# zabaras/deep-turbulence

Measured on AMD Instinct MI355X. Metric: flow-field samples/sec (fwd+log-det+bwd), 64x256x256x4; optimizer step: HipAdam (one-launch Adam, same update as torch.optim.Adam), higher is better.
Workload: dtype f32

## Files before the change

deep-turbulence_amd/csrc/tmg_common.h:

```cpp
#pragma once
#include <hip/hip_runtime.h>
#include <stdint.h>
#include <stdlib.h>
#include <atomic>

typedef float f32x4 __attribute__((ext_vector_type(4)));

__device__ __forceinline__ __amdgpu_buffer_rsrc_t tmg_make_rsrc(const void* base, unsigned bytes) {
    return __builtin_amdgcn_make_buffer_rsrc(const_cast<void*>(base), 0, (int)bytes, 0x00020000);
}
__device__ __forceinline__ float4 tmg_bload4(__amdgpu_buffer_rsrc_t rs, unsigned voff, unsigned soff) {
    const f32x4 v = __builtin_bit_cast(f32x4, __builtin_amdgcn_raw_buffer_load_b128(rs, (int)voff, (int)soff, 0));
    return make_float4(v[0], v[1], v[2], v[3]);
}

#define TMG_MAX_IN_SEG 3
#define TMG_MAX_OUT_SEG 3

struct TmgSeg {
    const float* p;
    int stride;
    int off;
    int n;
};
// ... 289 lines not shown
static inline int tmg_persistent_grid(int gy, int ntiles) {
    const int g = tmg_num_cus() / gy;
    return g > ntiles ? ntiles : (g < 1 ? 1 : g);
}

struct TmgSegList { int csum; bool vec4; };
template <typename SEG, typename PTRS>
static inline TmgSegList tmg_decode_segs(SEG* dst, int slots, PTRS ptrs, const int64_t* desc, int64_t n) {
    TmgSegList r{0, true};
    for (int i = 0; i < slots; ++i) {
        if (i >= n) { dst[i] = SEG{nullptr, 0, 0, 0}; continue; }
        dst[i] = SEG{(decltype(dst[i].p))ptrs[i], (int)desc[3 * i], (int)desc[3 * i + 1], (int)desc[3 * i + 2]};
        if (((dst[i].stride | dst[i].off | dst[i].n) & 3) || (((uintptr_t)ptrs[i]) & 15)) r.vec4 = false;
        r.csum += dst[i].n;
    }
    return r;
}
static inline TmgSegList tmg_decode_in(TmgSeg* dst, const void* const* ptrs, const int64_t* desc, int64_t n, int slots = TMG_MAX_IN_SEG) {
    return tmg_decode_segs(dst, slots, ptrs, desc, n);
}
static inline TmgSegList tmg_decode_out(TmgOSeg* dst, void* const* ptrs, const int64_t* desc, int64_t n, int slots = TMG_MAX_OUT_SEG) {
    return tmg_decode_segs(dst, slots, ptrs, desc, n);
}
static inline bool tmg_bad_seg_count(int64_t nin, int64_t nout) {
    return nin < 1 || nin > TMG_MAX_IN_SEG || nout < 1 || nout > TMG_MAX_OUT_SEG;
}
struct TmgD2 { int stride, off; };
static inline TmgD2 tmg_opt_d2(const void* p, const int64_t* d) { return p ? TmgD2{(int)d[0], (int)d[1]} : TmgD2{0, 0}; }

#define TMG_CHECK_LAUNCH()                          \
    do {                                            \
        hipError_t e__ = hipGetLastError();         \
        if (e__ != hipSuccess) return (int)e__;     \
    } while (0)
```

deep-turbulence_amd/csrc/tmg_conv.hip:

```cpp
#include "tmg_common.h"
#include <stdlib.h>

static __device__ float g_tmg_zero_page[64];

struct ConvP {
    TmgSeg in[TMG_MAX_IN_SEG];
    int nseg;
    int vec4;
    int B, Hin, Win, Hout, Wout;
    int ksize, stride;
    int Cin, Cin_pad, Cout, Cout_pad;
    const float* wpk;
    const float* bias;
    const float* kappa;
    const float* in_scale;
    const float* in_shift;
    int relu_in, pad_rep, relu_out, accumulate;
    TmgOSeg out[TMG_MAX_OUT_SEG];
    int nout;
    TmgSeg add;
    int TW_log2, TH;
    int KCH;
    int tiles_x, tiles_y;
    int ntiles, nchunks;
    int ovec4;
};

template <int MT, int NTW, int WM, int WN>
__global__ __launch_bounds__(256) void conv_mfma_kernel(ConvP p) {
    extern __shared__ __attribute__((aligned(16))) float lds[];
    const int tid = threadIdx.x, lane = tid & 63, wave = tid >> 6;
    const int wm = wave % WM, wn = wave / WM;
    const int li = lane & 15, q = lane >> 4;
    constexpr int MBLK = 16 * MT * WM;

    int t = blockIdx.x;
    const int tx = t % p.tiles_x;
    t /= p.tiles_x;
    const int ty = t % p.tiles_y;
    const int b = t / p.tiles_y;
    const int TWl = p.TW_log2, TW = 1 << TWl, TH = MBLK >> TWl;
    const int oy0 = ty * TH, ox0 = tx * TW;
    const int s = p.stride, halo = p.ksize >> 1;
    const int PW = s * (TW - 1) + 1 + 2 * halo, PH = s * (TH - 1) + 1 + 2 * halo;
    const int iy0 = s * oy0 - halo, ix0 = s * ox0 - halo;
    const int ntaps = p.ksize * p.ksize;
    const int KB = p.Cin_pad >> 4;

// ... 334 lines not shown
                if (store_only) {
#pragma unroll
                    for (int i = 0; i < MT; ++i) {
                        const int oy = oy0_ + (mrc[i] >> 16), ox = ox0_ + (mrc[i] & 0xffff);
                        if (oy < p.Hout && ox < p.Wout) {
                            const unsigned opx = (unsigned)(__umul24(b_ * p.Hout + oy, p.Wout) + ox);
#pragma unroll
                            for (int j = 0; j < NTW; ++j) {
                                const int n0 = (ntile0 + j) * 16 + 4 * qe;
                                if (n0 < p.Cout) {
                                    float v[4] = {acc[i][j][0], acc[i][j][1], acc[i][j][2], acc[i][j][3]};
                                    if (HB) { v[0] += biasq[HB ? j : 0].x; v[1] += biasq[HB ? j : 0].y; v[2] += biasq[HB ? j : 0].z; v[3] += biasq[HB ? j : 0].w; }
                                    if (PREADD && p.add.p) {
                                        const float4 a4 = addv[PREADD ? i : 0][PREADD ? j : 0];
                                        v[0] += a4.x; v[1] += a4.y; v[2] += a4.z; v[3] += a4.w;
                                    }
#pragma unroll
                                    for (int r = 0; r < 4; ++r) {
                                        v[r] *= osc;
                                        if (p.relu_out) v[r] = fmaxf(v[r], 0.f);
                                    }
                                    int nl = n0;
                                    TMG_PICK_OSEG(p.out, nl, op_, ostride, ooff)
                                    *reinterpret_cast<float4*>(op_ + (size_t)opx * (unsigned)ostride + ooff + nl) = make_float4(v[0], v[1], v[2], v[3]);
                                }
                            }
                        }
                    }
                } else
#pragma unroll
                for (int i = 0; i < MT; ++i) {
                    const int oy = oy0_ + (mrc[i] >> 16), ox = ox0_ + (mrc[i] & 0xffff);
                    if (oy < p.Hout && ox < p.Wout) {
                        const unsigned opx = (unsigned)(__umul24(b_ * p.Hout + oy, p.Wout) + ox);
#pragma unroll
                        for (int j = 0; j < NTW; ++j) {
                            const int n0 = (ntile0 + j) * 16 + 4 * qe;
                            if (n0 < p.Cout) {
                                float v[4] = {acc[i][j][0], acc[i][j][1], acc[i][j][2], acc[i][j][3]};
                                if (HB) {
                                    v[0] += biasq[HB ? j : 0].x; v[1] += biasq[HB ? j : 0].y; v[2] += biasq[HB ? j : 0].z; v[3] += biasq[HB ? j : 0].w;
                                } else if (p.bias) {
#pragma unroll
                                    for (int r = 0; r < 4; ++r) v[r] += (n0 + r < p.Cout) ? p.bias[n0 + r] : 0.f;
                                }
                                if (p.ovec4) {
                                    int nl = n0;
                                    TMG_PICK_OSEG(p.out, nl, op_, ostride, ooff)
                                    float4* dst = reinterpret_cast<float4*>(op_ + (size_t)opx * (unsigned)ostride + ooff + nl);
                                    if (p.add.p) {
                                        const float4 a4 = (PREADD) ? addv[PREADD ? i : 0][PREADD ? j : 0]
                                                                   : *reinterpret_cast<const float4*>(p.add.p + (size_t)opx * (unsigned)p.add.stride + p.add.off + n0);
                                        v[0] += a4.x; v[1] += a4.y; v[2] += a4.z; v[3] += a4.w;
                                    }
#pragma unroll
                                    for (int r = 0; r < 4; ++r) {
                                        v[r] *= osc;
                                        if (p.relu_out) v[r] = fmaxf(v[r], 0.f);
                                    }
                                    if (p.accumulate) {
                                        const float4 o4 = *dst;
                                        v[0] += o4.x; v[1] += o4.y; v[2] += o4.z; v[3] += o4.w;
                                    }
                                    *dst = make_float4(v[0], v[1], v[2], v[3]);
                                } else {
#pragma unroll
                                    for (int r = 0; r < 4; ++r) {
                                        const int n = n0 + r;
                                        if (n < p.Cout) {
                                            int nl = n;
                                            TMG_PICK_OSEG(p.out, nl, op_, ostride, ooff)
// ... 903 lines not shown
}

template <int MT, int NTW, int WM, int WN>
static int launch_fwd(const ConvP& p, int G, int gy, size_t lds_bytes, hipStream_t st, int64_t* plan) {
    if (plan) { fill_fwd_plan(plan, 0, MT, NTW, WM, WN, p, G, gy, lds_bytes); return 0; }
    TMG_LDS_OPTIN((&conv_fwd_kernel<MT, NTW, WM, WN>));
    const int kid = p.ksize == 1 ? 31 : 11 + (WM == 8 ? NTW - 1 : (WM == 4 ? NTW + 1 : NTW + 3));
    ProfScope prof(kid, 2.0 * p.B * p.Hout * p.Wout * (double)p.Cout * p.Cin * p.ksize * p.ksize, st);
    hipLaunchKernelGGL((conv_fwd_kernel<MT, NTW, WM, WN>), dim3(G, gy, 1), dim3(512), lds_bytes, st, p);
    TMG_CHECK_LAUNCH();
    return 0;
}

static int conv_fwd_lean(ConvP p, hipStream_t st, int64_t* plan) {
    if (p.stride != 1 || !p.vec4 || (p.Cin & 3) || (long)p.Hin * p.Win >= (1 << 24) || (long)p.B * p.Hout >= (1 << 24) ||
        p.Wout >= (1 << 24) || (long)p.B * p.Hout * p.Wout >= (1L << 32))
        return -100;
    for (int i = 0; i < p.nseg; ++i)
        if (p.in[i].stride >= (1 << 24) || (long)p.B * p.Hin * p.Win * p.in[i].stride >= (1L << 31)) return -100;
    p.ovec4 = (p.Cout & 3) == 0;
    for (int i = 0; i < p.nout; ++i)
        if (((p.out[i].stride | p.out[i].off | p.out[i].n) & 3) || (((uintptr_t)p.out[i].p) & 15)) p.ovec4 = 0;
    if (p.add.p && (((p.add.stride | p.add.off) & 3) || (((uintptr_t)p.add.p) & 15))) p.ovec4 = 0;
    const int ntt = p.Cout_pad >> 4;
    int WM, WN, NTW;
    if (ntt <= 4) { WM = 8; WN = 1; NTW = ntt; }
    else if (ntt <= 8) { WM = 4; WN = 2; NTW = ntt <= 6 ? 3 : 4; }
    else { WM = 2; WN = 4; NTW = ntt <= 12 ? 3 : 4; }
    const int gy = (ntt + WN * NTW - 1) / (WN * NTW);
    const long npix = (long)p.B * p.Hout * p.Wout;
    const int halo = p.ksize >> 1;
    for (int MT = 4; MT >= 1; MT >>= 1) {
        if (MT > 1 && (npix / (16 * MT * WM)) * gy < 256) continue;
        const int MBLK = 16 * MT * WM;
        int twl = ilog2_ceil(p.Wout);
        if (twl > 5) twl = 5;
        if (twl < 2) twl = 2;
        while ((1 << twl) > MBLK) --twl;
        while (twl < 5 && (MBLK >> twl) > p.Hout && (1 << twl) < p.Wout) ++twl;
        const int TW = 1 << twl, TH = MBLK >> twl;
        if (TH < 1) continue;
        const int PHPW = (TW + 2 * halo) * (TH + 2 * halo);
        int nchunks = (p.Cin_pad + 63) / 64, kch = 0;
        for (; nchunks <= p.Cin_pad / 16; ++nchunks) {
            kch = (((p.Cin_pad / 16) + nchunks - 1) / nchunks) * 16;
            const int k4p = kch <= 16 ? 4 : (kch <= 32 ? 8 : 16);
// ... 95 lines not shown

static int conv_fwd_impl(const void* const* in_ptrs, const int64_t* in_desc, int64_t nseg, const void* wpk, const void* bias,
                         const void* kappa, const void* in_scale, const void* in_shift, const void* add,
                         const int64_t* add_desc, void* const* out_ptrs, const int64_t* out_desc, int64_t nout,
                         const int64_t* dims, hipStream_t st, int64_t* plan) {
    ConvP p;
    const TmgD2 ad = tmg_opt_d2(add, add_desc);
    p.add = TmgSeg{(const float*)add, ad.stride, ad.off, 0};
    p.nseg = (int)nseg;
    const TmgSegList si = tmg_decode_in(p.in, in_ptrs, in_desc, nseg);
    p.vec4 = si.vec4;
    p.B = (int)dims[0]; p.Hin = (int)dims[1]; p.Win = (int)dims[2]; p.Hout = (int)dims[3]; p.Wout = (int)dims[4];
    p.ksize = (int)dims[5]; p.stride = (int)dims[6]; p.Cin = (int)dims[7]; p.Cout = (int)dims[8];
    p.relu_in = (int)dims[9]; p.pad_rep = (int)dims[10]; p.relu_out = (int)dims[11]; p.accumulate = (int)dims[12];
    if (p.ksize != 1 && p.ksize != 3) return -2;
    if (si.csum != p.Cin || tmg_bad_seg_count(nseg, nout)) return -3;
    p.Cin_pad = (p.Cin + 15) & ~15;
    p.Cout_pad = (p.Cout + 15) & ~15;
    p.wpk = (const float*)wpk; p.bias = (const float*)bias; p.kappa = (const float*)kappa;
    p.in_scale = (const float*)in_scale; p.in_shift = (const float*)in_shift;
    p.nout = (int)nout;
    if (tmg_decode_out(p.out, out_ptrs, out_desc, nout).csum != p.Cout) return -4;

    {
        const int rc = conv_fwd_lean(p, st, plan);
        if (rc != -100) return rc;
    }

    const int ntt = p.Cout_pad >> 4;
    int WM, WN, NTW;
    if (ntt <= 4) { WM = 4; WN = 1; NTW = ntt; }
    else if (ntt <= 6) { WM = 2; WN = 2; NTW = 3; }
    else if (ntt <= 8) { WM = 2; WN = 2; NTW = 4; }
    else if (ntt <= 12) { WM = 1; WN = 4; NTW = 3; }
    else { WM = 1; WN = 4; NTW = 4; }
    const int gy = (ntt + WN * NTW - 1) / (WN * NTW);
    int MT = 4;
    while (MT > 1) {
        const long npix = (long)p.B * p.Hout * p.Wout;
        if ((npix / (16 * MT * WM)) * gy >= 512) break;
        MT >>= 1;
    }
    const int MBLK = 16 * MT * WM;
    int twl = ilog2_ceil(p.Wout);
    if (twl > 5) twl = 5;
    if (twl < 2) twl = 2;
    while ((1 << twl) > MBLK) --twl;
    while (twl < 5 && (MBLK >> twl) > p.Hout && (1 << twl) < p.Wout) ++twl;
    p.TW_log2 = twl;
    const int TW = 1 << twl;
// ... 365 lines not shown
```

deep-turbulence_amd/csrc/tmg_wino.hip:

```cpp
#include "tmg_common.h"
#include <stdlib.h>
#include <type_traits>

struct WinoP {
    TmgSeg in[TMG_MAX_IN_SEG];
    int nseg;
    int B, Hin, Win;
    int Cin, Cin_pad, Cout, Npad;
    const float* U;
    const float* bias;
    int relu_in, pad_rep;
    TmgOSeg out[TMG_MAX_OUT_SEG];
    int tiles_x, tiles_y, ntiles;
    int nchunks;
};

__global__ void wino_pack_kernel(const float* __restrict__ w, float* __restrict__ U, int Cout, int Cin, int K, int N, int Kpad, int Npad, int mode) {
    const size_t total = (size_t)Kpad * Npad;
    for (size_t i = blockIdx.x * (size_t)blockDim.x + threadIdx.x; i < total; i += (size_t)gridDim.x * blockDim.x) {
        const int c16 = i & 15;
        size_t r = i >> 4;
        const int n = r % Npad;
        const int kb = r / Npad;
        const int k = kb * 16 + c16;
        float g[3][3];
#pragma unroll
        for (int a = 0; a < 3; ++a)
#pragma unroll
            for (int b = 0; b < 3; ++b) {
                float v = 0.f;
                if (k < K && n < N) v = mode == 0 ? w[((size_t)n * Cin + k) * 9 + a * 3 + b] : w[((size_t)k * Cin + n) * 9 + (2 - a) * 3 + (2 - b)];
                g[a][b] = v;
            }
        float t[4][3];
#pragma unroll
// ... 242 lines not shown
                    TMG_WN_POSITION
                };
#define TMG_WN_P(I) one_position(std::integral_constant<int, I>{});
                TMG_WN_P(0) TMG_WN_P(1) TMG_WN_P(2) TMG_WN_P(3) TMG_WN_P(4) TMG_WN_P(5) TMG_WN_P(6) TMG_WN_P(7)
                TMG_WN_P(8) TMG_WN_P(9) TMG_WN_P(10) TMG_WN_P(11) TMG_WN_P(12) TMG_WN_P(13) TMG_WN_P(14) TMG_WN_P(15)
#undef TMG_WN_P
#undef TMG_WN_LOADB
            }
            if (cm + 1 == nchunks) {
                int t_ = tm;
                const int tx_ = t_ % p.tiles_x; t_ /= p.tiles_x;
                const int ty_ = t_ % p.tiles_y;
                const int b_ = t_ / p.tiles_y;
#pragma unroll
                for (int m = 0; m < 2; ++m) {
                    const int wt = 16 * m + li;
                    const int oyb = ty_ * TH + 2 * (wt >> 3), oxb = tx_ * TW + 2 * (wt & 7);
#pragma unroll
                    for (int n = 0; n < NPW; ++n) {
                        const int n0 = (ntile0 + n) * 16 + 4 * q;
                        if (ntile0 + n < ntt && n0 < p.Cout) {
                            int nl = n0;
                            TMG_PICK_OSEG(p.out, nl, optr, ostride, ooff)
#pragma unroll
                            for (int o = 0; o < 4; ++o) {
                                const int oy = oyb + (o >> 1), ox = oxb + (o & 1);
                                if (oy < p.Hin && ox < p.Win) {
                                    const unsigned opx = ((unsigned)b_ * (unsigned)p.Hin + (unsigned)oy) * (unsigned)p.Win + (unsigned)ox;
                                    *reinterpret_cast<float4*>(optr + (size_t)opx * (unsigned)ostride + ooff + nl) =
                                        make_float4(Y[o][m][n][0], Y[o][m][n][1], Y[o][m][n][2], Y[o][m][n][3]);
                                }
                            }
                        }
                    }
                }
#pragma unroll
                for (int o = 0; o < 4; ++o)
#pragma unroll
                    for (int m = 0; m < 2; ++m)
#pragma unroll
                        for (int n = 0; n < NPW; ++n) Y[o][m][n] = bvr[n];
                cm = 0; tm += G;
            } else {
                ++cm;
            }
        }
// ... 151 lines not shown
                    af[0][m] = v4[(pos * VPL + m * 16 * VS) / 4];
                    af[1][m] = v4[(pos * VPL + m * 16 * VS + 16) / 4];
                }
                __builtin_amdgcn_sched_barrier(0);
                TMG_WN_POSITION
            }
        }
#undef TMG_WN_LOADB
        if (cm + 1 == nchunks) {
            int t_ = tm;
            const int tx_ = t_ % p.tiles_x; t_ /= p.tiles_x;
            const int ty_ = t_ % p.tiles_y;
            const int b_ = t_ / p.tiles_y;
#pragma unroll
            for (int m = 0; m < 2; ++m) {
                const int wt = 16 * m + li;
                const int oyb = ty_ * TH + 2 * (wt >> 3), oxb = tx_ * TW + 2 * (wt & 7);
#pragma unroll
                for (int n = 0; n < NPW; ++n) {
                    const int n0 = (ntile0 + n) * 16 + 4 * q;
                    if (ntile0 + n < ntt && n0 < p.Cout) {
                        int nl = n0;
                        TMG_PICK_OSEG(p.out, nl, optr, ostride, ooff)
#pragma unroll
                        for (int o = 0; o < 4; ++o) {
                            const int oy = oyb + (o >> 1), ox = oxb + (o & 1);
                            if (oy < p.Hin && ox < p.Win) {
                                const unsigned opx = ((unsigned)b_ * (unsigned)p.Hin + (unsigned)oy) * (unsigned)p.Win + (unsigned)ox;
                                *reinterpret_cast<float4*>(optr + (size_t)opx * (unsigned)ostride + ooff + nl) =
                                    make_float4(Y[o][m][n][0], Y[o][m][n][1], Y[o][m][n][2], Y[o][m][n][3]);
                            }
                        }
                    }
                }
            }
#pragma unroll
            for (int o = 0; o < 4; ++o)
#pragma unroll
                for (int m = 0; m < 2; ++m)
#pragma unroll
                    for (int n = 0; n < NPW; ++n) Y[o][m][n] = bvr[n];
            cm = 0; tm += G;
        } else {
            ++cm;
        }
    }
}

template <typename P>
static int wino_fwd_setup(P& p, const void* const* in_ptrs, const int64_t* in_desc, int64_t nseg, const void* U, const void* bias,
                          void* const* out_ptrs, const int64_t* out_desc, int64_t nout, const int64_t* dims, int cin_granule, bool narrow) {
    p.nseg = (int)nseg;
    if (tmg_bad_seg_count(nseg, nout)) return -3;
    const TmgSegList si = tmg_decode_in(p.in, in_ptrs, in_desc, nseg), so = tmg_decode_out(p.out, out_ptrs, out_desc, nout);
    p.B = (int)dims[0]; p.Hin = (int)dims[1]; p.Win = (int)dims[2]; p.Cin = (int)dims[3]; p.Cout = (int)dims[4];
    p.relu_in = (int)dims[5]; p.pad_rep = (int)dims[6];
    if (si.csum != p.Cin || so.csum != p.Cout) return -3;
    bool ok = si.vec4 && so.vec4 && !(p.Cout & 3) && !(p.Cin & 3);
    if (narrow ? (p.Cout > 48 || p.Cin < 64) : p.Cout < 64) ok = false;
    if (bias && (((uintptr_t)bias) & 15)) ok = false;
    if (!ok) return -100;
    p.Cin_pad = (p.Cin + cin_granule - 1) & ~(cin_granule - 1);
    p.Npad = (p.Cout + 15) & ~15;
    p.U = (const float*)U; p.bias = (const float*)bias;
    p.tiles_x = (p.Win + 15) / 16; p.tiles_y = (p.Hin + 7) / 8;
    p.ntiles = p.B * p.tiles_x * p.tiles_y;
    p.nchunks = (p.Cin_pad + 31) / 32;
    if (p.ntiles <= 0) return 0;
    if ((long long)p.B * p.Hin * p.Win >= (1LL << 31)) return -100;
    return 1;
}

#define TMG_WINO_FWD_PLAN_N 13
template <typename P>
static void fill_wino_fwd_plan(int64_t* plan, int kernel, int npw, const P& p, int gx, int gy, size_t lds_bytes) {
    const int64_t v[TMG_WINO_FWD_PLAN_N] = {kernel, npw, p.Cin_pad, p.nchunks, (p.Cin_pad - 32 * (p.nchunks - 1) + 15) / 16, p.Npad / 16, p.tiles_x,
                                            p.tiles_y, p.ntiles, gx, gy, (p.ntiles + gx - 1) / gx, (int64_t)lds_bytes};
    for (int i = 0; i < TMG_WINO_FWD_PLAN_N; ++i) plan[i] = v[i];
}

// ... 317 lines not shown
                for (int m = 0; m < 2; ++m)
#pragma unroll
                    for (int n = 0; n < NPW; ++n) TMG_W3_YUPD(15, m, n)
#undef TMG_W3_YUPD
#undef TMG_W3_LOADB
            }
            if (cm + 1 == nch) {
                int t_ = tm;
                const int tx_ = t_ % p.tiles_x; t_ /= p.tiles_x;
                const int ty_ = t_ % p.tiles_y;
                const int b_ = t_ / p.tiles_y;
                int lie = li, qe = q;
                asm volatile("" : "+v"(lie), "+v"(qe));
#pragma unroll
                for (int m = 0; m < 2; ++m) {
                    const int wt = 16 * m + lie;
                    const int oyb = ty_ * TH + 2 * (wt >> 3), oxb = tx_ * TW + 2 * (wt & 7);
#pragma unroll
                    for (int n = 0; n < NPW; ++n) {
                        const int n0 = (ntile0 + n) * 16 + 4 * qe;
                        if (ntile0 + n < ntt && n0 < p.Cout) {
                            int nl = n0;
                            TMG_PICK_OSEG(p.out, nl, optr, ostride, ooff)
#pragma unroll
                            for (int o = 0; o < 4; ++o) {
                                const int oy = oyb + (o >> 1), ox = oxb + (o & 1);
                                if (oy < p.Hin && ox < p.Win) {
                                    const unsigned opx = ((unsigned)b_ * (unsigned)p.Hin + (unsigned)oy) * (unsigned)p.Win + (unsigned)ox;
                                    __builtin_nontemporal_store(Y[o][m][n],
                                                                reinterpret_cast<f32x4*>(optr + (size_t)opx * (unsigned)ostride + ooff + nl));
                                }
                            }
                        }
                    }
                }
#pragma unroll
                for (int o = 0; o < 4; ++o)
#pragma unroll
                    for (int m = 0; m < 2; ++m)
#pragma unroll
                        for (int n = 0; n < NPW; ++n) Y[o][m][n] = bvr[n];
                cm = 0; tm += G;
            } else {
                ++cm;
            }
        }
// ... 767 lines not shown
```

deep-turbulence_amd/tmg_hip.py:

```python
import ctypes
import os
import weakref
import subprocess
import sys

import torch

_HERE = os.path.dirname(os.path.abspath(__file__))
LIB_PATH = os.path.join(_HERE, "libtmglow_hip.so")
CSRC = os.path.join(_HERE, "csrc")
SOURCES = ["tmg_conv.hip", "tmg_pointwise.hip", "tmg_physics.hip", "tmg_mix16.hip", "tmg_coupling.hip", "tmg_wino.hip", "tmg_thin.hip", "tmg_glue.hip", "tmg_ensemble.hip", "tmg_spectrum.hip", "tmg_scores.hip", "tmg_tspec.hip", "tmg_quant.hip", "tmg_gram.hip", "tmg_sfun.hip", "tmg_event.hip", "tmg_pdf.hip", "tmg_pod.hip", "tmg_phase.hip", "tmg_spod.hip"]
NO_PACKED_F32 = ["tmg_wino.hip", "tmg_conv.hip", "tmg_coupling.hip", "tmg_thin.hip", "tmg_mix16.hip", "tmg_spectrum.hip", "tmg_tspec.hip",
                 "tmg_pod.hip", "tmg_spod.hip"]
_lib = None

c_i64 = ctypes.c_int64
c_vp = ctypes.c_void_p

EXPORTS = [
    "tmg_conv_pack", "tmg_conv_pack_map", "tmg_conv_fwd", "tmg_conv_fwd_add", "tmg_affine_bwd_scaled", "tmg_c1_fwd_add", "tmg_conv_wgrad", "tmg_conv_wgrad_ws_floats", "tmg_conv_rep_border_fix", "tmg_conv_dgrad_direct",
    "tmg_affine_apply", "tmg_affine_apply_pass", "tmg_bn_finalize", "tmg_affine_bwd", "tmg_lstm_pointwise_fwd", "tmg_lstm_pointwise_bwd", "tmg_gauss_fwd",
    "tmg_gauss_bwd", "tmg_checker", "tmg_upsample_fwd", "tmg_upsample_bwd", "tmg_chan_reduce", "tmg_bn_bwd_apply",
    "tmg_phys_fwd", "tmg_phys_rms", "tmg_phys_bwd", "tmg_conv_wgrad_grouped", "tmg_conv_wgrad_grouped_ws_floats", "tmg_conv_pack_batched", "tmg_masked_add", "tmg_c1x2_fwd", "tmg_c1_fwd", "tmg_c1_bwd", "tmg_dense2_bwd", "tmg_dkappa", "tmg_prof_enable", "tmg_prof_collect", "tmg_mix_f16", "tmg_phys_bwd_dev", "tmg_coupling_fwd", "tmg_coupling_bwd",
    "tmg_conv_wino_pack", "tmg_conv_wino_fwd", "tmg_conv_wino_narrow", "tmg_conv_wino_wgrad", "tmg_conv_wino_wgrad_ws_floats", "tmg_mix_f32", "tmg_lu_fold_fwd", "tmg_lu_fold_bwd", "tmg_lu_fold_bwd_split", "tmg_level_finish", "tmg_conv_wgrad_thin_grouped", "tmg_mix_wgrad_grouped", "tmg_layer_planes", "tmg_conv_wino_wgrad_grouped", "tmg_conv_wino_wgrad_grouped_ws_floats", "tmg_adam_step", "tmg_chan_moments", "tmg_bn_finalize64", "tmg_mix_f32_affine_fwd", "tmg_mix_f32_affine_bwd", "tmg_conv_pack_many", "tmg_pad_halves", "tmg_coupling_fwd_halves", "tmg_coupling_bwd_halves", "tmg_fill_i64", "tmg_conv_wino_pack3", "tmg_conv_wino_fwd3", "tmg_mat_inverse", "tmg_gauss_sample", "tmg_reverse_loss_fwd", "tmg_reverse_loss_bwd", "tmg_sum_terms", "tmg_vec_sum", "tmg_level_pack", "tmg_spread2", "tmg_phys_fields", "tmg_phys_fields_bwd",
# ... 141 lines not shown
    if t.is_cuda and t.device.index != torch.cuda.current_device():
        raise RuntimeError("TM-Glow HIP op called with a tensor on %s while the current device is cuda:%d: wrap the call in "
                           "`with torch.cuda.device(t.device):` (or torch.cuda.set_device once per process)"
                           % (t.device, torch.cuda.current_device()))


def nhwc(x):
    check_act(x)
    check_device(x)
    return x.permute(0, 2, 3, 1).contiguous()


def nchw(t):
    return t.permute(0, 3, 1, 2)


def _segs(tensors):
    d = [seg(t) for t in tensors]
    ptrs = (c_vp * len(d))(*[x[0] for x in d])
    desc = (c_i64 * (3 * len(d)))(*[v for x in d for v in (x[1], x[2], x[3])])
    return ptrs, desc, len(d)


def _d2(t):
    return (c_i64 * 2)(seg(t)[1] if t is not None else 0, 0)


def _i64(*v):
    return (c_i64 * len(v))(*[int(x) for x in v])


def _flts(vals):
    return (ctypes.c_float * len(vals))(*[float(v) for v in vals])


def _launched(rc, name):
    if rc == -100:
        return False
    _chk(rc, name)
    return True


def _packed_numel(mode, ce, Cout, k):
    K, N = (ce, Cout) if mode == 0 else (Cout, ce)
    return k * k * ((K + 15) // 16 * 16) * ((N + 15) // 16 * 16)

# ... 79 lines not shown
        op = (c_vp * len(ws))(*[v.data_ptr() for v in views])
        _chk(lib().tmg_conv_pack_many(wp, op, _i64(*desc), c_i64(len(ws)), _stream()), "tmg_conv_pack_many")
        outs += views
    return outs


def conv_pack_batched(w, mode, cin_eff=0, cmap=None):
    check_act(w)
    w = w.contiguous()
    N_, Cout, Cin, k, _ = w.shape
    ce = int(cin_eff) if cmap is not None else max(int(cin_eff), Cin)
    wpk = torch.empty((N_, _packed_numel(mode, ce, Cout, k)), device=w.device, dtype=torch.float32)
    m = cmap if cmap is not None else (Cin, 0x7fffffff, 0)
    _chk(lib().tmg_conv_pack_batched(_ptr(w), _ptr(wpk), c_i64(N_), c_i64(Cout), c_i64(Cin), c_i64(ce), c_i64(k), c_i64(mode), _i64(*m),
                                     _stream()), "tmg_conv_pack_batched")
    return wpk


def conv_fwd(inputs, wpk, Cout, ksize, stride, outs, bias=None, kappa=None, in_scale=None, in_shift=None, relu_in=False,
             pad_rep=False, relu_out=False, accumulate=False, add=None):
    B, Hin, Win, _ = inputs[0].shape
    Hout, Wout = outs[0].shape[1], outs[0].shape[2]
    ip, idesc, n_in = _segs(inputs)
    op, odesc, n_out = _segs(outs)
    Cin = sum(t.shape[3] for t in inputs)
    assert sum(t.shape[3] for t in outs) == Cout
    dims = _i64(B, Hin, Win, Hout, Wout, ksize, stride, Cin, Cout, relu_in, pad_rep, relu_out, accumulate)
    if add is not None:
        _chk(lib().tmg_conv_fwd_add(ip, idesc, c_i64(n_in), _ptr(wpk), _ptr(bias), _ptr(kappa), _ptr(in_scale), _ptr(in_shift), _ptr(add),
                                    _d2(add), op, odesc, c_i64(n_out), dims, _stream()), "tmg_conv_fwd_add")
        return
    _chk(lib().tmg_conv_fwd(ip, idesc, c_i64(n_in), _ptr(wpk), _ptr(bias), _ptr(kappa), _ptr(in_scale), _ptr(in_shift), op, odesc,
                            c_i64(n_out), dims, _stream()), "tmg_conv_fwd")


def wino_eligible(Cin, Cout, ksize, stride):
    return ksize == 3 and stride == 1 and Cout >= 64 and Cout % 4 == 0 and Cin % 4 == 0 and Cin >= 16


def wino_narrow_eligible(Cin, Cout):
    return Cout <= 48 and Cout % 4 == 0 and Cin % 4 == 0 and Cin >= 64


def conv_wino_pack(w, mode=0, nvalid=0):
    Cout, Cin = w.shape[0], w.shape[1]
    assert w.shape[2] == 3 and w.shape[3] == 3
    w = w.contiguous()
# ... 7 lines not shown


def set_winograd_precision(kind):
    if kind not in ("f32", "bf16x3"):
        raise ValueError("Winograd precision must be 'f32' or 'bf16x3', got %r" % (kind,))
    _WINO_PRECISION[0] = kind


def winograd_precision():
    return _WINO_PRECISION[0]


def conv_wino_pack3(w, mode=0, nvalid=0):
    Cout, Cin = w.shape[0], w.shape[1]
    assert w.shape[2] == 3 and w.shape[3] == 3
    w = w.contiguous()
    K, N = (Cin, Cout) if mode == 0 else (Cout, nvalid if 0 < nvalid < Cin else Cin)
    U = torch.empty(16 * ((K + 31) // 32 * 32) * ((N + 15) // 16 * 16) * 3, device=w.device, dtype=torch.int16)
    _chk(lib().tmg_conv_wino_pack3(_ptr(w), _ptr(U), c_i64(Cout), c_i64(Cin), c_i64(mode), c_i64(nvalid), _stream()), "tmg_conv_wino_pack3")
    return U


def _wino_fwd(name, inputs, U, Cout, outs, bias, *flags):
    if isinstance(outs, torch.Tensor):
        outs = [outs]
    B, Hin, Win, _ = inputs[0].shape
    ip, idesc, n_in = _segs(inputs)
    op, odesc, n_out = _segs(outs)
    Cin = sum(t.shape[3] for t in inputs)
    assert sum(t.shape[3] for t in outs) == Cout and outs[0].shape[1] == Hin and outs[0].shape[2] == Win
    return _launched(getattr(lib(), name)(ip, idesc, c_i64(n_in), _ptr(U), _ptr(bias), op, odesc, c_i64(n_out),
                                          _i64(B, Hin, Win, Cin, Cout, *flags), _stream()), name)


def conv_wino_fwd3(inputs, U, Cout, outs, bias=None, relu_in=False, pad_rep=False):
    return _wino_fwd("tmg_conv_wino_fwd3", inputs, U, Cout, outs, bias, relu_in, pad_rep)


def conv_wino_narrow(inputs, U, Cout, outs, bias=None, relu_in=False, pad_rep=False, relu_out=False):
    return _wino_fwd("tmg_conv_wino_narrow", inputs, U, Cout, outs, bias, relu_in, pad_rep, relu_out)


def conv_wino_fwd(inputs, U, Cout, outs, bias=None, relu_in=False, pad_rep=False):
    return _wino_fwd("tmg_conv_wino_fwd", inputs, U, Cout, outs, bias, relu_in, pad_rep)


def conv3x3_auto(inputs, weight, Cout, outs, bias=None, relu_in=False, pad_rep=False, relu_out=False, dgrad=False, nvalid=0):
    Cin = sum(t.shape[3] for t in inputs)
    mode = 1 if dgrad else 0
    if not relu_out and wino_eligible(Cin, Cout, 3, 1):
        if (_WINO_PRECISION[0] == "bf16x3"
                and conv_wino_fwd3(inputs, conv_wino_pack3(weight, mode, nvalid), Cout, outs, bias=bias, relu_in=relu_in, pad_rep=pad_rep)):
            return None
        if conv_wino_fwd(inputs, conv_wino_pack(weight, mode, nvalid), Cout, outs, bias=bias, relu_in=relu_in, pad_rep=pad_rep):
            return None
    if wino_narrow_eligible(Cin, Cout):
        if conv_wino_narrow(inputs, conv_wino_pack(weight, mode, nvalid), Cout, outs, bias=bias, relu_in=relu_in, pad_rep=pad_rep,
                            relu_out=relu_out):
            return None
    wpk = conv_pack(weight, mode, nvalid, (nvalid, 1 << 30, 0)) if (dgrad and nvalid) else conv_pack(weight, mode)
    conv_fwd(inputs, wpk, Cout, 3, 1, outs, bias=bias, relu_in=relu_in, pad_rep=pad_rep, relu_out=relu_out)
    return wpk


_WS = {}


def workspace(nfloats, device):
    if torch.cuda.is_current_stream_capturing():
        return torch.empty(max(int(nfloats), 1), device=device, dtype=torch.float32)
    key = (device.index, torch._C._cuda_getCurrentRawStream(torch._C._cuda_getDevice()))
    buf = _WS.get(key)
    if buf is None or buf.numel() < nfloats:
        buf = torch.empty(max(int(nfloats), 1 << 20), device=device, dtype=torch.float32)
        _WS[key] = buf
    return buf


_WINO_WGRAD_CIN_MIN = 32
# ... 1011 lines not shown
```

deep-turbulence_amd/tmg_ops.py:

```python
import collections
import math
import numbers

import os
import threading
import weakref

import torch

import tmg_hip as H

LOG5 = math.log(5.0)
LOG4 = math.log(4.0)
SPLIT_LIMITS = (-2.0, LOG5, -2.0, LOG5)
TOP_LIMITS = (0.0, 0.0, -10.0, LOG5)


class _ZeroPool:
    CHUNK = 8 << 20
    LIMIT = 2 << 20

    def __init__(self):
        self.lock = threading.Lock()
        self.cur = {}
# ... 908 lines not shown
    return dx


_Level = collections.namedtuple("_Level", "NL NLp C ch Cc cin reverse fuse split rec w1s w2s wzs bzs kps")
_LevelBwd = collections.namedtuple("_LevelBwd", "g Wm PZt PMt DH DD quad_last grouped zc_kw wg_in mix_wg dWz dBz dW1 dW2 dWm dbm DDp")


def _level(wts, C, Cc, reverse):
    NL = len(wts) // 5
    ch = C // 2
    fuse = 8 <= C <= 32 and ch % 4 == 0 and all(w.is_contiguous() for w in wts)
    split = fuse and reverse and C in (16, 32)
    rec = _RECOMPUTE[0] and fuse and reverse and C <= 64
    return _Level(NL, (NL + 3) // 4 * 4, C, ch, Cc, ch + Cc, reverse, fuse, split, rec,
                  wts[0::5], wts[1::5], wts[2::5], wts[3::5], wts[4::5])


class LevelCouplingFn(torch.autograd.Function):

    @staticmethod
    def _cond_parts(L, cond, Wcat):
        bhw, dev = cond.shape[:3], cond.device
        Wzc, Wdc = Wcat[:L.NL * L.C], Wcat[L.NL * L.C:]
        Hc = empty(bhw + (L.NL * L.C,), dev)
        H.conv3x3_auto([cond], Wzc, L.NL * L.C, [Hc], relu_in=True, pad_rep=True)
        Dc = empty(bhw + (2 * L.NLp,), dev)
        H.conv_fwd([cond], H.conv_pack(Wdc, 0), 2 * L.NLp, 3, 1, [Dc], relu_in=True)
        if math.prod(bhw) >= int(os.environ.get("TMG_LAYER_PLANES_MIN", 1 << 17)):
            Dc = H.layer_planes(Dc)
            dc_of = lambda k: (Dc[k][..., 0:1], Dc[k][..., 1:2])
        else:
            dc_of = lambda k: (Dc[..., 2 * k:2 * k + 1], Dc[..., 2 * k + 1:2 * k + 2])
        return Hc, Dc, dc_of

    @staticmethod
    def _level_operands(L, dev):
        NL, NLp, C, ch, Cc, cin = L[:6]
        layers = list(zip(L.w1s, L.w2s, L.wzs, L.bzs, L.kps))
        Wz = empty((NL, C, cin + 2, 3, 3), dev)
        Wcat = empty((NL * C + 2 * NLp, Cc, 3, 3), dev)
        Bz = empty((NL, C), dev)
        Kp = empty(NL, dev)
        if all(w.is_contiguous() and w.dtype == torch.float32 for ws in layers for w in ws) and os.environ.get("TMG_NO_LEVEL_PACK") is None:
            tab = H._segment_table([[w.data_ptr() for w in ws] for ws in layers], dev)
            H.level_pack(tab, Wz, Wcat, Bz, Kp, NL, NLp, C, ch, Cc)
            return Wz, Wcat, Bz, Kp
        torch.stack(L.wzs, out=Wz)
        Wcat[:NL * C] = Wz[:, :, ch:cin].reshape(NL * C, Cc, 3, 3)
        Wdc = Wcat[NL * C:].view(NLp, 2, Cc, 3, 3)
        Wdc[NL:].zero_()
        Wdc[:NL, 0] = torch.stack(L.w1s)[:, 0, ch:cin]
        Wdc[:NL, 1] = torch.stack(L.w2s)[:, 0, ch:cin]
        torch.stack(L.bzs, out=Bz)
        torch.stack([kp.reshape(()) for kp in L.kps], out=Kp)
        return Wz, Wcat, Bz, Kp

    @staticmethod
    def _growth(L, k, x1, dc_of):
        D = empty(x1.shape[:3] + (4,), x1.device)
        add1, add2 = dc_of(k)
        H.c1x2_fwd([x1], L.w1s[k], L.w2s[k], D, w_rows=L.ch, w2_d1_row=L.cin, add1=add1, add2=add2)
        return D

    @staticmethod
    def _fwd_fused(L, k, cur, Wm, bm, PM, Hc, dc_of, logdet):
        C, ch, reverse = L.C, L.ch, L.reverse
        bhw, dev = Hc.shape[:3], Hc.device
        tin = cur if reverse else _mix_fwd(cur, Wm[k], bm[k], PM[k])
        t1 = H._halves(tin)[0]
        D = LevelCouplingFn._growth(L, k, t1, dc_of)
        if L.split and k != 0:
            out = (empty(bhw + (ch,), dev), empty(bhw + (ch,), dev))
        else:
            out = empty(bhw + (C,), dev)
        r = empty(bhw + (ch,), dev)
        y2 = empty(bhw + (ch,), dev) if reverse else None
        ok = H.coupling_fwd(tin, out, r, y2, D, Hc[..., k * C:(k + 1) * C], L.wzs[k], L.bzs[k], L.kps[k], Wm[k] if reverse else None,
                            bm[k] if reverse else None, logdet, reverse, L.cin)
        assert ok
        if L.rec:
            return out, None
        return out, ((tin, D, r, [t1, y2]) if reverse else (tin, D, r, out, cur))

    @staticmethod
    def _fwd_wide(L, k, cur, Wm, bm, PM, PZ, Hc, dc_of, logdet, mixaff):
        C, ch, reverse = L.C, L.ch, L.reverse
        bhw, dev = Hc.shape[:3], Hc.device
        tin = cur if reverse else _mix_fwd(cur, Wm[k], bm[k], PM[k])
        x1 = tin[..., :ch]
        if ch % 4 == 0:
            D = LevelCouplingFn._growth(L, k, x1, dc_of)
        else:
            D = empty(bhw + (4,), dev)
            add1, add2 = dc_of(k)
            H.c1_fwd([x1], L.w1s[k], D[..., 0:1], relu_in=True, w_rows=ch, fill4=True, add=add1)
            H.c1_fwd([x1, D], L.w2s[k], D[..., 1:2], relu_in=True, w_rows=ch + 1, w_split=ch, w_gap=L.Cc, add=add2)
        hh = empty(bhw + (C,), dev)
        H.conv_fwd([x1, D], PZ[k], C, 3, 1, [hh], bias=L.bzs[k], kappa=L.kps[k], relu_in=True, pad_rep=True, add=Hc[..., k * C:(k + 1) * C])
        r = empty(bhw + (ch,), dev)
        if mixaff:
            y2 = empty(bhw + (ch,), dev)
            out = empty(bhw + (C,), dev)
            if H.mix_affine_fwd(tin, hh, Wm[k], bm[k], out, r, y2, logdet):
                return out, (tin, D, r, [x1, y2])
        y = empty(bhw + (C,), dev)
        H.affine_apply(hh, tin[..., ch:], y[..., ch:], r, logdet, reverse, x1=x1, y1=y[..., :ch])
        return (_mix_fwd(y, Wm[k], bm[k], PM[k]) if reverse else y), (tin, D, r, y) + (() if reverse else (cur,))

    @staticmethod
    def forward(ctx, x, cond, Wm, bm, reverse, *wts):
        x = x if x.stride(3) == 1 else x.contiguous()
        cond = cond.contiguous()
        L = _level(wts, x.shape[3], cond.shape[3], reverse)
        NL, C, ch = L.NL, L.C, L.ch
        dev = x.device
        Wz, Wcat, Bz, Kp = LevelCouplingFn._level_operands(L, dev)
        Hc, Dc, dc_of = LevelCouplingFn._cond_parts(L, cond, Wcat)
        logdet = zeros(x.shape[0], dev)
        PZ = H.conv_pack_batched(Wz, 0, ch + 4, (ch + 2, ch, L.Cc))
        PM = H.conv_pack_batched(Wm.reshape(NL, C, C, 1, 1), 0)
        mixaff = (reverse and C in (64, 128) and Wm.is_contiguous() and bm.is_contiguous()
                  and os.environ.get("TMG_NO_MIX_AFFINE") is None)
        saved = [None] * NL
        cur = x
        for k in (range(NL - 1, -1, -1) if reverse else range(NL)):
            if L.fuse:
                cur, saved[k] = LevelCouplingFn._fwd_fused(L, k, cur, Wm, bm, PM, Hc, dc_of, logdet)
            else:
                cur, saved[k] = LevelCouplingFn._fwd_wide(L, k, cur, Wm, bm, PM, PZ, Hc, dc_of, logdet, mixaff)
        del Hc, Dc
        ctx.saved = saved
        ctx.rec_out = cur if L.rec else None
        ctx.level = L
        ctx.save_for_backward(cond, Wm, bm, Wz, Wcat, Bz, Kp, *wts)
        return cur.view(cur.shape), logdet

    @staticmethod
    def _rebuild(L, R, k):
        Hc, dc_of, Winv, binv, ld_dummy, out = R
        C, ch = L.C, L.ch
        u = _mix_fwd(out, Winv[k], binv[k])
        t1 = u[..., :ch]
        D = LevelCouplingFn._growth(L, k, t1, dc_of)
        tin = empty(u.shape, u.device)
        r = empty(t1.shape, u.device)
        ok = H.coupling_fwd(u, tin, r, None, D, Hc[..., k * C:(k + 1) * C], L.wzs[k], L.bzs[k], L.kps[k], None, None, ld_dummy, False, L.cin)
        assert ok
        R[-1] = tin
        return tin, D, r, [t1, u[..., ch:]]

    @staticmethod
    def _zero_conv_wgrad(L, S, k, x1D, now=False):
        if S.grouped and not now:
            S.wg_in[k] = x1D
        else:
            H.conv_wgrad(x1D, S.DH[..., k * L.C:(k + 1) * L.C], S.dWz[k], S.dBz[k], 3, 1, **S.zc_kw)

    @staticmethod
    def _mix_wgrad(L, S, k, x, dy, now=False):
        x = x if isinstance(x, list) else [x]
        if S.grouped and not now:
            S.mix_wg[k] = (x, dy)
        else:
            H.conv_wgrad(x, dy if torch.is_tensor(dy) else torch.cat(list(dy), 3), S.dWm[k], S.dbm[k], 1, 1)

    @staticmethod
    def _layer_mix_bwd(L, S, k, x, dy):
        dx = _mix_dgrad(dy, S.Wm[k], S.PMt[k])
        LevelCouplingFn._mix_wgrad(L, S, k, x, dy)
# ... 135 lines not shown
        ctx.saved = None
        dy = dy.contiguous()
        bhw, dev = dy.shape[:3], dy.device
        g = dld.contiguous() if dld is not None else None
        dWz, dW1, dW2, dBz, dWm, dbm = carve(dev, (NL, C, cin + 2, 3, 3), (NL, 1, cin, 3, 3), (NL, 1, cin + 1, 3, 3), (NL, C), (NL, C, C),
                                             (NL, C))
        DH = empty(bhw + (NL * C,), dev)
        DDp = None
        if math.prod(bhw) >= int(os.environ.get("TMG_LAYER_PLANES_MIN", 1 << 17)):
            DDp, DD = empty((NL,) + bhw + (2,), dev), None
        else:
            DD = empty(bhw + (2 * NLp,), dev)
        quad_last = NLp - NL == 1
        if DD is not None and NLp - NL > 1:
            DD[..., 2 * NL:].zero_()
        grouped = NL > 1 and ch + 4 <= 132
        PZt = H.conv_pack_batched(Wz, 1, ch + 4, (ch + 2, ch, Cc))
        PMt = H.conv_pack_batched(Wm.reshape(NL, C, C, 1, 1), 1)
        zc_kw = dict(relu_in=True, pad_rep=True, cin_dst=cin + 2, cin_valid=ch + 2, ci_split=ch, ci_off0=0, ci_off1=Cc)
        S = _LevelBwd(g, Wm, PZt, PMt, DH, DD, quad_last, grouped, zc_kw, [None] * NL, [None] * NL if grouped else None, dWz, dBz, dW1, dW2,
                      dWm, dbm, DDp)
        R = None
        if ctx.rec_out is not None:
            Hc_r, Dc_r, dc_of_r = LevelCouplingFn._cond_parts(L, cond, Wcat)
            Winv, binv = H.mat_inverse(Wm, bm)
            R = [Hc_r, dc_of_r, Winv, binv, zeros(bhw[0], dev), ctx.rec_out]
        ctx.rec_out = None
        if not L.fuse:
            step = LevelCouplingFn._bwd_wide
        else:
            step = LevelCouplingFn._bwd_fused_generative if L.reverse else LevelCouplingFn._bwd_fused_density
        dcur = dy
        for k in (range(NL) if L.reverse else range(NL - 1, -1, -1)):
            dcur = step(L, S, k, dcur, *LevelCouplingFn._activations(L, R, saved, k))
        tmpX = LevelCouplingFn._grouped_wgrads(L, S) if grouped else None
        if DDp is not None:
            S = S._replace(DD=H.layer_unplanes(DDp, 2 * NLp), DDp=None)
        Gc, tmpC = LevelCouplingFn._cond_bwd(L, S, cond, Wcat)
        dK = LevelCouplingFn._finish(L, S, Wz, Bz, Kp, tmpX, tmpC)
        grads = []
        for k in range(NL):
            grads += [dW1[k], dW2[k], dWz[k], dBz[k], dK[k].reshape(L.kps[k].shape)]
        return (dcur, Gc, dWm, dbm, None) + _defer(wts, grads)


class LevelMixFoldFn(torch.autograd.Function):

    @staticmethod
    def forward(ctx, meta, *params):
# ... 1608 lines not shown
```

Baseline: 1519.

## Write conditioning conv output as per-layer 16-channel NHWC planes

The conditioning 3x3 conv that produces Hc for every coupling layer can now write its output as a stack of contiguous 16-channel planes, one per layer, instead of one wide interleaved NHWC tensor. Direct and Winograd conv kernels gain an otile offset so each 16-channel output tile goes to its own plane. Each coupling layer then reads a dense 16-channel tensor rather than a strided slice of a wide one, which should improve locality and vectorised access in the consumers. Narrow-Winograd and non-lean paths reject plane output, so some shapes may fall back to slower kernels.

```diff
diff --git a/deep-turbulence_amd/csrc/tmg_common.h b/deep-turbulence_amd/csrc/tmg_common.h
--- a/deep-turbulence_amd/csrc/tmg_common.h
+++ b/deep-turbulence_amd/csrc/tmg_common.h
@@ -335,6 +335,12 @@
 static inline TmgSegList tmg_decode_out(TmgOSeg* dst, void* const* ptrs, const int64_t* desc, int64_t n, int slots = TMG_MAX_OUT_SEG) {
     return tmg_decode_segs(dst, slots, ptrs, desc, n);
 }
+static inline long long tmg_out_planes(TmgOSeg* out, const int64_t* desc, int64_t nout, long long npix) {
+    if (nout != 1 || desc[0] >= desc[2]) return 0;
+    if (desc[0] != 16 || (desc[2] & 15) || desc[1] < npix * 16 || (desc[1] & 3) || (desc[2] >> 4) * desc[1] >= (1LL << 31)) return -1;
+    out[0].off = 0;
+    return (long long)desc[1];
+}
 static inline bool tmg_bad_seg_count(int64_t nin, int64_t nout) {
     return nin < 1 || nin > TMG_MAX_IN_SEG || nout < 1 || nout > TMG_MAX_OUT_SEG;
 }
diff --git a/deep-turbulence_amd/csrc/tmg_conv.hip b/deep-turbulence_amd/csrc/tmg_conv.hip
--- a/deep-turbulence_amd/csrc/tmg_conv.hip
+++ b/deep-turbulence_amd/csrc/tmg_conv.hip
@@ -24,6 +24,7 @@
     int tiles_x, tiles_y;
     int ntiles, nchunks;
     int ovec4;
+    int otile;
 };
 
 template <int MT, int NTW, int WM, int WN>
@@ -404,6 +405,7 @@
                                     }
                                     int nl = n0;
                                     TMG_PICK_OSEG(p.out, nl, op_, ostride, ooff)
+                                    nl += (ntile0 + j) * p.otile;
                                     *reinterpret_cast<float4*>(op_ + (size_t)opx * (unsigned)ostride + ooff + nl) = make_float4(v[0], v[1], v[2], v[3]);
                                 }
                             }
@@ -429,6 +431,7 @@
                                 if (p.ovec4) {
                                     int nl = n0;
                                     TMG_PICK_OSEG(p.out, nl, op_, ostride, ooff)
+                                    nl += (ntile0 + j) * p.otile;
                                     float4* dst = reinterpret_cast<float4*>(op_ + (size_t)opx * (unsigned)ostride + ooff + nl);
                                     if (p.add.p) {
                                         const float4 a4 = (PREADD) ? addv[PREADD ? i : 0][PREADD ? j : 0]
@@ -1378,6 +1381,7 @@
     for (int i = 0; i < p.nout; ++i)
         if (((p.out[i].stride | p.out[i].off | p.out[i].n) & 3) || (((uintptr_t)p.out[i].p) & 15)) p.ovec4 = 0;
     if (p.add.p && (((p.add.stride | p.add.off) & 3) || (((uintptr_t)p.add.p) & 15))) p.ovec4 = 0;
+    if (p.otile && !p.ovec4) return -100;
     const int ntt = p.Cout_pad >> 4;
     int WM, WN, NTW;
     if (ntt <= 4) { WM = 8; WN = 1; NTW = ntt; }
@@ -1519,10 +1523,14 @@
     p.nout = (int)nout;
     if (tmg_decode_out(p.out, out_ptrs, out_desc, nout).csum != p.Cout) return -4;
 
+    const long long oplane = tmg_out_planes(p.out, out_desc, nout, (long long)p.B * p.Hout * p.Wout);
+    if (oplane < 0) return -4;
+    p.otile = oplane ? (int)(oplane - 16) : 0;
     {
         const int rc = conv_fwd_lean(p, st, plan);
         if (rc != -100) return rc;
     }
+    if (oplane) return -8;
 
     const int ntt = p.Cout_pad >> 4;
     int WM, WN, NTW;
diff --git a/deep-turbulence_amd/csrc/tmg_wino.hip b/deep-turbulence_amd/csrc/tmg_wino.hip
--- a/deep-turbulence_amd/csrc/tmg_wino.hip
+++ b/deep-turbulence_amd/csrc/tmg_wino.hip
@@ -11,6 +11,7 @@
     const float* bias;
     int relu_in, pad_rep;
     TmgOSeg out[TMG_MAX_OUT_SEG];
+    int otile;
     int tiles_x, tiles_y, ntiles;
     int nchunks;
 };
@@ -299,6 +300,7 @@
                         if (ntile0 + n < ntt && n0 < p.Cout) {
                             int nl = n0;
                             TMG_PICK_OSEG(p.out, nl, optr, ostride, ooff)
+                            nl += (ntile0 + n) * p.otile;
 #pragma unroll
                             for (int o = 0; o < 4; ++o) {
                                 const int oy = oyb + (o >> 1), ox = oxb + (o & 1);
@@ -496,6 +498,7 @@
                     if (ntile0 + n < ntt && n0 < p.Cout) {
                         int nl = n0;
                         TMG_PICK_OSEG(p.out, nl, optr, ostride, ooff)
+                        nl += (ntile0 + n) * p.otile;
 #pragma unroll
                         for (int o = 0; o < 4; ++o) {
                             const int oy = oyb + (o >> 1), ox = oxb + (o & 1);
@@ -530,6 +533,10 @@
     p.B = (int)dims[0]; p.Hin = (int)dims[1]; p.Win = (int)dims[2]; p.Cin = (int)dims[3]; p.Cout = (int)dims[4];
     p.relu_in = (int)dims[5]; p.pad_rep = (int)dims[6];
     if (si.csum != p.Cin || so.csum != p.Cout) return -3;
+    const long long oplane = tmg_out_planes(p.out, out_desc, nout, (long long)p.B * p.Hin * p.Win);
+    if (oplane < 0) return -3;
+    if constexpr (std::is_same<P, WinoP>::value) p.otile = oplane ? (int)(oplane - 16) : 0;
+    else if (oplane) return -3;
     bool ok = si.vec4 && so.vec4 && !(p.Cout & 3) && !(p.Cin & 3);
     if (narrow ? (p.Cout > 48 || p.Cin < 64) : p.Cout < 64) ok = false;
     if (bias && (((uintptr_t)bias) & 15)) ok = false;
@@ -893,6 +900,7 @@
                         if (ntile0 + n < ntt && n0 < p.Cout) {
                             int nl = n0;
                             TMG_PICK_OSEG(p.out, nl, optr, ostride, ooff)
+                            nl += (ntile0 + n) * p.otile;
 #pragma unroll
                             for (int o = 0; o < 4; ++o) {
                                 const int oy = oyb + (o >> 1), ox = oxb + (o & 1);
diff --git a/deep-turbulence_amd/tmg_hip.py b/deep-turbulence_amd/tmg_hip.py
--- a/deep-turbulence_amd/tmg_hip.py
+++ b/deep-turbulence_amd/tmg_hip.py
@@ -187,6 +187,17 @@
     return ptrs, desc, len(d)
 
 
+def _osegs(outs):
+    if isinstance(outs, torch.Tensor) and outs.dim() == 5:
+        check_act(outs)
+        NT, B, H, W, c = outs.shape
+        if not (c == 16 and NT > 1 and outs[0].is_contiguous() and outs.stride(0) >= B * H * W * 16 and outs.stride(0) % 4 == 0
+                and NT * outs.stride(0) < 1 << 31):
+            raise RuntimeError("not a stack of 16-channel NHWC planes: shape %s strides %s" % (tuple(outs.shape), outs.stride()))
+        return (c_vp * 1)(outs.data_ptr()), (c_i64 * 3)(16, outs.stride(0), NT * 16), 1
+    return _segs(outs)
+
+
 def _d2(t):
     return (c_i64 * 2)(seg(t)[1] if t is not None else 0, 0)
 
@@ -312,7 +323,7 @@
     B, Hin, Win, _ = inputs[0].shape
     Hout, Wout = outs[0].shape[1], outs[0].shape[2]
     ip, idesc, n_in = _segs(inputs)
-    op, odesc, n_out = _segs(outs)
+    op, odesc, n_out = _osegs(outs)
     Cin = sum(t.shape[3] for t in inputs)
     assert sum(t.shape[3] for t in outs) == Cout
     dims = _i64(B, Hin, Win, Hout, Wout, ksize, stride, Cin, Cout, relu_in, pad_rep, relu_out, accumulate)
@@ -366,11 +377,11 @@
 
 
 def _wino_fwd(name, inputs, U, Cout, outs, bias, *flags):
-    if isinstance(outs, torch.Tensor):
+    if isinstance(outs, torch.Tensor) and outs.dim() == 4:
         outs = [outs]
     B, Hin, Win, _ = inputs[0].shape
     ip, idesc, n_in = _segs(inputs)
-    op, odesc, n_out = _segs(outs)
+    op, odesc, n_out = _osegs(outs)
     Cin = sum(t.shape[3] for t in inputs)
     assert sum(t.shape[3] for t in outs) == Cout and outs[0].shape[1] == Hin and outs[0].shape[2] == Win
     return _launched(getattr(lib(), name)(ip, idesc, c_i64(n_in), _ptr(U), _ptr(bias), op, odesc, c_i64(n_out),
@@ -398,7 +409,8 @@
             return None
         if conv_wino_fwd(inputs, conv_wino_pack(weight, mode, nvalid), Cout, outs, bias=bias, relu_in=relu_in, pad_rep=pad_rep):
             return None
-    if wino_narrow_eligible(Cin, Cout):
+    planes = isinstance(outs, torch.Tensor) and outs.dim() == 5
+    if wino_narrow_eligible(Cin, Cout) and not planes:
         if conv_wino_narrow(inputs, conv_wino_pack(weight, mode, nvalid), Cout, outs, bias=bias, relu_in=relu_in, pad_rep=pad_rep,
                             relu_out=relu_out):
             return None
diff --git a/deep-turbulence_amd/tmg_ops.py b/deep-turbulence_amd/tmg_ops.py
--- a/deep-turbulence_amd/tmg_ops.py
+++ b/deep-turbulence_amd/tmg_ops.py
@@ -954,16 +954,23 @@
     def _cond_parts(L, cond, Wcat):
         bhw, dev = cond.shape[:3], cond.device
         Wzc, Wdc = Wcat[:L.NL * L.C], Wcat[L.NL * L.C:]
-        Hc = empty(bhw + (L.NL * L.C,), dev)
-        H.conv3x3_auto([cond], Wzc, L.NL * L.C, [Hc], relu_in=True, pad_rep=True)
+        planes = math.prod(bhw) >= int(os.environ.get("TMG_LAYER_PLANES_MIN", 1 << 17))
+        if planes and L.C == 16 and L.NL > 1 and L.Cc % 4 == 0:
+            Hc = empty((L.NL,) + bhw + (L.C,), dev)
+            H.conv3x3_auto([cond], Wzc, L.NL * L.C, Hc, relu_in=True, pad_rep=True)
+            hc_of = lambda k: Hc[k]
+        else:
+            Hc = empty(bhw + (L.NL * L.C,), dev)
+            H.conv3x3_auto([cond], Wzc, L.NL * L.C, [Hc], relu_in=True, pad_rep=True)
+            hc_of = lambda k: Hc[..., k * L.C:(k + 1) * L.C]
         Dc = empty(bhw + (2 * L.NLp,), dev)
         H.conv_fwd([cond], H.conv_pack(Wdc, 0), 2 * L.NLp, 3, 1, [Dc], relu_in=True)
-        if math.prod(bhw) >= int(os.environ.get("TMG_LAYER_PLANES_MIN", 1 << 17)):
+        if planes:
             Dc = H.layer_planes(Dc)
             dc_of = lambda k: (Dc[k][..., 0:1], Dc[k][..., 1:2])
         else:
             dc_of = lambda k: (Dc[..., 2 * k:2 * k + 1], Dc[..., 2 * k + 1:2 * k + 2])
-        return Hc, Dc, dc_of
+        return hc_of, dc_of
 
     @staticmethod
     def _level_operands(L, dev):
@@ -995,11 +1002,11 @@
         return D
 
     @staticmethod
-    def _fwd_fused(L, k, cur, Wm, bm, PM, Hc, dc_of, logdet):
+    def _fwd_fused(L, k, cur, Wm, bm, PM, hc_of, dc_of, logdet):
         C, ch, reverse = L.C, L.ch, L.reverse
-        bhw, dev = Hc.shape[:3], Hc.device
         tin = cur if reverse else _mix_fwd(cur, Wm[k], bm[k], PM[k])
         t1 = H._halves(tin)[0]
+        bhw, dev = t1.shape[:3], t1.device
         D = LevelCouplingFn._growth(L, k, t1, dc_of)
         if L.split and k != 0:
             out = (empty(bhw + (ch,), dev), empty(bhw + (ch,), dev))
@@ -1007,7 +1014,7 @@
             out = empty(bhw + (C,), dev)
         r = empty(bhw + (ch,), dev)
         y2 = empty(bhw + (ch,), dev) if reverse else None
-        ok = H.coupling_fwd(tin, out, r, y2, D, Hc[..., k * C:(k + 1) * C], L.wzs[k], L.bzs[k], L.kps[k], Wm[k] if reverse else None,
+        ok = H.coupling_fwd(tin, out, r, y2, D, hc_of(k), L.wzs[k], L.bzs[k], L.kps[k], Wm[k] if reverse else None,
                             bm[k] if reverse else None, logdet, reverse, L.cin)
         assert ok
         if L.rec:
@@ -1015,9 +1022,9 @@
         return out, ((tin, D, r, [t1, y2]) if reverse else (tin, D, r, out, cur))
 
     @staticmethod
-    def _fwd_wide(L, k, cur, Wm, bm, PM, PZ, Hc, dc_of, logdet, mixaff):
+    def _fwd_wide(L, k, cur, Wm, bm, PM, PZ, hc_of, dc_of, logdet, mixaff):
         C, ch, reverse = L.C, L.ch, L.reverse
-        bhw, dev = Hc.shape[:3], Hc.device
+        bhw, dev = cur.shape[:3], cur.device
         tin = cur if reverse else _mix_fwd(cur, Wm[k], bm[k], PM[k])
         x1 = tin[..., :ch]
         if ch % 4 == 0:
@@ -1028,7 +1035,7 @@
             H.c1_fwd([x1], L.w1s[k], D[..., 0:1], relu_in=True, w_rows=ch, fill4=True, add=add1)
             H.c1_fwd([x1, D], L.w2s[k], D[..., 1:2], relu_in=True, w_rows=ch + 1, w_split=ch, w_gap=L.Cc, add=add2)
         hh = empty(bhw + (C,), dev)
-        H.conv_fwd([x1, D], PZ[k], C, 3, 1, [hh], bias=L.bzs[k], kappa=L.kps[k], relu_in=True, pad_rep=True, add=Hc[..., k * C:(k + 1) * C])
+        H.conv_fwd([x1, D], PZ[k], C, 3, 1, [hh], bias=L.bzs[k], kappa=L.kps[k], relu_in=True, pad_rep=True, add=hc_of(k))
         r = empty(bhw + (ch,), dev)
         if mixaff:
             y2 = empty(bhw + (ch,), dev)
@@ -1047,7 +1054,7 @@
         NL, C, ch = L.NL, L.C, L.ch
         dev = x.device
         Wz, Wcat, Bz, Kp = LevelCouplingFn._level_operands(L, dev)
-        Hc, Dc, dc_of = LevelCouplingFn._cond_parts(L, cond, Wcat)
+        hc_of, dc_of = LevelCouplingFn._cond_parts(L, cond, Wcat)
         logdet = zeros(x.shape[0], dev)
         PZ = H.conv_pack_batched(Wz, 0, ch + 4, (ch + 2, ch, L.Cc))
         PM = H.conv_pack_batched(Wm.reshape(NL, C, C, 1, 1), 0)
@@ -1057,10 +1064,10 @@
         cur = x
         for k in (range(NL - 1, -1, -1) if reverse else range(NL)):
             if L.fuse:
-                cur, saved[k] = LevelCouplingFn._fwd_fused(L, k, cur, Wm, bm, PM, Hc, dc_of, logdet)
+                cur, saved[k] = LevelCouplingFn._fwd_fused(L, k, cur, Wm, bm, PM, hc_of, dc_of, logdet)
             else:
-                cur, saved[k] = LevelCouplingFn._fwd_wide(L, k, cur, Wm, bm, PM, PZ, Hc, dc_of, logdet, mixaff)
-        del Hc, Dc
+                cur, saved[k] = LevelCouplingFn._fwd_wide(L, k, cur, Wm, bm, PM, PZ, hc_of, dc_of, logdet, mixaff)
+        del hc_of, dc_of
         ctx.saved = saved
         ctx.rec_out = cur if L.rec else None
         ctx.level = L
@@ -1069,14 +1076,14 @@
 
     @staticmethod
     def _rebuild(L, R, k):
-        Hc, dc_of, Winv, binv, ld_dummy, out = R
-        C, ch = L.C, L.ch
+        hc_of, dc_of, Winv, binv, ld_dummy, out = R
+        ch = L.ch
         u = _mix_fwd(out, Winv[k], binv[k])
         t1 = u[..., :ch]
         D = LevelCouplingFn._growth(L, k, t1, dc_of)
         tin = empty(u.shape, u.device)
         r = empty(t1.shape, u.device)
-        ok = H.coupling_fwd(u, tin, r, None, D, Hc[..., k * C:(k + 1) * C], L.wzs[k], L.bzs[k], L.kps[k], None, None, ld_dummy, False, L.cin)
+        ok = H.coupling_fwd(u, tin, r, None, D, hc_of(k), L.wzs[k], L.bzs[k], L.kps[k], None, None, ld_dummy, False, L.cin)
         assert ok
         R[-1] = tin
         return tin, D, r, [t1, u[..., ch:]]
@@ -1258,9 +1265,9 @@
                       dWm, dbm, DDp)
         R = None
         if ctx.rec_out is not None:
-            Hc_r, Dc_r, dc_of_r = LevelCouplingFn._cond_parts(L, cond, Wcat)
+            hc_of_r, dc_of_r = LevelCouplingFn._cond_parts(L, cond, Wcat)
             Winv, binv = H.mat_inverse(Wm, bm)
-            R = [Hc_r, dc_of_r, Winv, binv, zeros(bhw[0], dev), ctx.rec_out]
+            R = [hc_of_r, dc_of_r, Winv, binv, zeros(bhw[0], dev), ctx.rec_out]
         ctx.rec_out = None
         if not L.fuse:
             step = LevelCouplingFn._bwd_wide
```

After: 1515. No clear change (-0.2%).
